# crowsonkb/style_transfer2

Hardware: AMD Instinct MI355X
Metric: style-transfer iters/sec @1024px VGG19 (higher is better)
Workload: dtype f32; 1 GPU; configs[1]: 1024x1024 single image per GPU, VGG19 to conv5_1, content conv4_2 + 5 style layers, adam fp32, 500 iterations per image; jobs=1, parallelism=independent jobs, 1 per GPU, no collective (replicas)

## Files before the change

style_transfer2_amd/csrc/conv3x3_winograd.hip:

```cpp
#include <hip/hip_runtime.h>
#include <stdint.h>
#include <stdlib.h>
#include <string.h>
#include <type_traits>
#include "st2_kernels.h"
#include "env.h"

namespace st2 {

typedef float f32x16 __attribute__((ext_vector_type(16)));
typedef float f32x4 __attribute__((ext_vector_type(4)));


constexpr int WN_CH = 8;
constexpr int WN_IW = 40;
constexpr int WN_V = 4 * 16 * 64;

size_t wino_pack_floats(int K, int M) { return (size_t)((M + 127) / 128 * 4) * (K / 2) * 1024; }

static void wino_pack(const float* w, int Cout, int Cin, bool dgrad, float* dst)
{
    const int K = dgrad ? Cout : Cin, M = dgrad ? Cin : Cout, nkp = K / 2;
    memset(dst, 0, wino_pack_floats(K, M) * sizeof(float));
    static const double G[4][3] = {{1, 0, 0}, {0.5, 0.5, 0.5}, {0.5, -0.5, 0.5}, {0, 0, 1}};
    for (int m = 0; m < M; ++m)
        for (int k = 0; k < K; ++k) {
            double g[3][3], t[4][3], u[4][4];
            for (int tap = 0; tap < 9; ++tap)
                g[tap / 3][tap % 3] = dgrad ? w[((size_t)k * Cin + m) * 9 + (8 - tap)] : w[((size_t)m * Cin + k) * 9 + tap];
            for (int i = 0; i < 4; ++i)
                for (int j = 0; j < 3; ++j) t[i][j] = G[i][0] * g[0][j] + G[i][1] * g[1][j] + G[i][2] * g[2][j];
            for (int i = 0; i < 4; ++i)
                for (int j = 0; j < 4; ++j) u[i][j] = t[i][0] * G[j][0] + t[i][1] * G[j][1] + t[i][2] * G[j][2];
            const size_t base = ((size_t)(m / 32) * nkp + k / 2) * 1024;
            const int lane = (k & 1) * 32 + (m & 31);
            for (int pos = 0; pos < 16; ++pos)
                dst[base + ((size_t)(pos >> 2) * 64 + lane) * 4 + (pos & 3)] = (float)u[pos >> 2][pos & 3];
        }
}
void pack_wino_weights_fwd(const float* w, int Cout, int Cin, float* dst) { wino_pack(w, Cout, Cin, false, dst); }
void pack_wino_weights_dgrad(const float* w, int Cout, int Cin, float* dst) { wino_pack(w, Cout, Cin, true, dst); }

struct WinoKArgs {
    const float* in; const float4* upack; const float* bias; float* out;
    const float* mask_src; const float* inject;
    int K, M, H, W, nch, tiles_x, tiles_y, n_mtiles, relu;
    unsigned in_bytes, u_bytes;
    float* pool_out; int pool_h, pool_w;
    unsigned char* pool_amap;
    const unsigned char* unpool_amap; unsigned amap_bytes; int ph, pw;
    int splits; float* scratch;
    unsigned long long* stamps;
};

typedef __attribute__((address_space(3))) void* lptr_t;
constexpr unsigned kOOB = 0xffffffffu;

__device__ __forceinline__ float f4c(const float4& v, int i) { return i == 0 ? v.x : i == 1 ? v.y : i == 2 ? v.z : v.w; }

template <int EPI, bool RS> struct WinoEpiOps {
    static constexpr bool E_FWD = EPI == 1 || EPI == 2, E_MASK = EPI == 3;
    static constexpr int NEB = RS ? 2 : 4;
    static constexpr int NG = E_MASK ? 2 * NEB : NEB;
    static constexpr int UNDER = NG < 4 ? NG : 4;
    int mw, dm0, odd;
    bool live, has_inj;
    unsigned row0, plane4, out_bytes;
    float mk[E_MASK ? NEB : 1][E_MASK ? 4 : 1][4], ij[E_FWD ? 1 : NEB][E_FWD ? 1 : 4][4], bs[E_FWD ? NEB : 1][E_FWD ? 4 : 1];

    __device__ __forceinline__ void init(const WinoKArgs& a, int lane, int yw, int x0, int m0, int ph, unsigned plane)
    {
        odd = lane & 1;
        const int gy = yw + 2 * ((lane & 31) >> 4) + odd;
        const int gx4 = x0 + 2 * (lane & 14);
        live = gx4 < a.W && gy < a.H;
        mw = m0 + 4 * (lane >> 5);
        dm0 = RS ? 16 * ph : 0;
        has_inj = a.inject != nullptr;
        plane4 = plane * 4u;
        out_bytes = (unsigned)a.M * plane4;
// ... 49 lines not shown
    constexpr int IN_ROWS = PROWS + 2;
    constexpr int IW = QUAD ? WN_IW : 64;
    constexpr int COL0 = QUAD ? 3 : 0;
    constexpr int PLANE = IN_ROWS * IW;
    constexpr int UP_ROWS = PROWS / 2 + 2, UP_COLS = 24;
    constexpr int UP_PLANE = UP_ROWS * UP_COLS;
    constexpr int UP_F = WN_CH * UP_PLANE;
    constexpr int UP_FQ = UP_F / 256, UP_AQ = UP_F / 256;
    static_assert(!UNPOOL || (UP_F % 256 == 0 && NW == 4), "unpool staging is a whole number of wave-DMAs");
    constexpr int N_RAW = UNPOOL ? UP_F + UP_F / 4 : WN_CH * PLANE;
    constexpr int I_PER_WAVE = UNPOOL ? (UP_FQ + UP_AQ + NW - 1) / NW
                             : QUAD ? (N_RAW / 4 + 64 * NW - 1) / (64 * NW) : WN_CH * IN_ROWS / 4;
    constexpr int RAW = UNPOOL ? 1024 : QUAD ? I_PER_WAVE * NW * 256 : N_RAW;
    static_assert(QUAD || (WN_CH * IN_ROWS) % 4 == 0, "rows divide over the four waves");

    __shared__ __attribute__((aligned(16))) float raw_s[2][RAW];
    __shared__ __attribute__((aligned(16))) float v_s[2][TG][WN_V];
    __shared__ __attribute__((aligned(16))) float x8_own[W8 ? 8 * 8 * 64 * 4 : 4];
    static_assert(!H4 || 4 * 8 * 64 * 4 <= 2 * TG * WN_V, "H4: the exchange buffer fits the V images");
    float* const x8_s = H4 ? &v_s[0][0][0] : x8_own;

    const int tid = threadIdx.x;
    const int lane = tid & 63;
    const int wave = __builtin_amdgcn_readfirstlane(tid >> 6);
    const int wave_m = W8 ? (wave & 3) : H4 ? (wave & 1) : wave / TG, wave_g = RS ? 0 : wave % TG;
    const int ph = W8 ? wave >> 2 : H4 ? wave >> 1 : wave_g;

    const int nwg = gridDim.x / a.splits;
    const int split = blockIdx.x / nwg, orig = blockIdx.x - split * nwg;
    const int nch = a.nch / a.splits, c_first = split * nch;
    const int xcd = orig & 7, q = nwg >> 3, r = nwg & 7;
    const int logical = (xcd < r ? xcd * (q + 1) : r * (q + 1) + (xcd - r) * q) + (orig >> 3);
    const int n_pt = a.tiles_x * a.tiles_y;
    const int mt = logical / n_pt;
    const int pt = logical - mt * n_pt;
    const int tx = pt % a.tiles_x;
    const int ty = pt / a.tiles_x;
    const int y0 = ty * PROWS, x0 = tx * 32;
    const unsigned plane = (unsigned)a.H * a.W;
    const int nkp = a.K >> 1;

    const unsigned long long t_begin = DIAG ? __builtin_amdgcn_s_memtime() : 0ull;

    const __amdgpu_buffer_rsrc_t rs_i = __builtin_amdgcn_make_buffer_rsrc((void*)a.in, 0, a.in_bytes, 0x00020000);
    const __amdgpu_buffer_rsrc_t rs_a = __builtin_amdgcn_make_buffer_rsrc((void*)(UNPOOL ? a.unpool_amap : nullptr), 0, UNPOOL ? a.amap_bytes : 0u, 0x00020000);
    const unsigned pplane = UNPOOL ? (unsigned)a.ph * a.pw : 0u;
    unsigned ioff[QUAD ? I_PER_WAVE : 1];
    if (UNPOOL) {
#pragma unroll
        for (int t = 0; t < I_PER_WAVE; ++t) {
            const int piece = wave + NW * t;
            const bool bytes = piece >= UP_FQ;
            const int e = ((bytes ? piece - UP_FQ : piece) * 64 + lane) * 4;
            const int c = e / UP_PLANE;
            const int rem = e - c * UP_PLANE;
            const int rr = rem / UP_COLS;
            const int col = rem - rr * UP_COLS;
            const int gy = (y0 >> 1) - 1 + rr, gx = (x0 >> 1) - 4 + col;
            const bool ok = piece < UP_FQ + UP_AQ && gy >= 0 && gy < a.ph && gx >= 0 && gx + 3 < a.pw;
            ioff[t] = ok ? ((unsigned)((BIG && !bytes ? 0 : c_first * WN_CH) + c) * pplane + (unsigned)gy * a.pw + gx) * (bytes ? 1u : 4u) : kOOB;
        }
    } else if (QUAD) {
#pragma unroll
        for (int t = 0; t < I_PER_WAVE; ++t) {
            const int e = ((wave + NW * t) * 64 + lane) * 4;
            const int c = e / PLANE;
            const int rem = e - c * PLANE;
            const int rr = rem / IW;
            const int col = rem - rr * IW;
            const int gy = y0 - 1 + rr, gx = x0 - 4 + col;
            const bool ok = e < N_RAW && gy >= 0 && gy < a.H && gx >= 0 && gx + 3 < a.W;
            ioff[t] = ok ? ((unsigned)((BIG ? 0 : c_first * WN_CH) + c) * plane + (unsigned)gy * a.W + gx) * 4u : kOOB;
        }
    } else {
        const int gx = x0 - 1 + lane;
        ioff[0] = (lane < 34 && gx >= 0 && gx < a.W) ? (unsigned)gx * 4u : kOOB;
    }
    auto dma_raw = [&](int ch, int buf) {
        const __amdgpu_buffer_rsrc_t rs_c = BIG ? __builtin_amdgcn_make_buffer_rsrc(
            (void*)(a.in + (size_t)(c_first + ch) * WN_CH * (UNPOOL ? pplane : plane)), 0, a.in_bytes, 0x00020000) : rs_i;
        if (UNPOOL) {
#pragma unroll
            for (int t = 0; t < I_PER_WAVE; ++t) {
                const int piece = wave + NW * t;
                if (piece < UP_FQ) {
                    const unsigned vo = (ioff[t] == kOOB || BIG) ? ioff[t] : ioff[t] + (unsigned)ch * WN_CH * pplane * 4u;
                    __builtin_amdgcn_raw_ptr_buffer_load_lds(rs_c, (lptr_t)(raw_s[buf] + piece * 256), 16, vo, 0, 0, 0);
                } else if (piece < UP_FQ + UP_AQ) {
                    const unsigned vo = ioff[t] == kOOB ? kOOB : ioff[t] + (unsigned)ch * WN_CH * pplane;
                    __builtin_amdgcn_raw_ptr_buffer_load_lds(rs_a, (lptr_t)(raw_s[buf] + UP_F + (piece - UP_FQ) * 64), 4, vo, 0, 0, 0);
                }
            }
        } else if (QUAD) {
            const unsigned coff = BIG ? 0u : (unsigned)ch * WN_CH * plane * 4u;
#pragma unroll
            for (int t = 0; t < I_PER_WAVE; ++t) {
                const unsigned vo = ioff[t] == kOOB ? kOOB : ioff[t] + coff;
                __builtin_amdgcn_raw_ptr_buffer_load_lds(rs_c, (lptr_t)(raw_s[buf] + (wave + NW * t) * 256), 16, vo, 0, 0, 0);
            }
        } else {
#pragma unroll
            for (int t = 0; t < I_PER_WAVE; ++t) {
                const int row = wave + 4 * t;
                const int c = row / IN_ROWS, gy = y0 - 1 + (row - c * IN_ROWS);
                const bool row_ok = gy >= 0 && gy < a.H;
                const unsigned base = ((unsigned)((c_first + ch) * WN_CH + c) * plane + (unsigned)(row_ok ? gy : 0) * a.W) * 4u;
                const unsigned vo = (row_ok && ioff[0] != kOOB) ? ioff[0] + base : kOOB;
                __builtin_amdgcn_raw_ptr_buffer_load_lds(rs_i, (lptr_t)(raw_s[buf] + row * 64), 4, vo, 0, 0, 0);
            }
        }
    };

    const int xt = tid & 31, xch = (tid >> 5) & 7;
    const int x_raw = UNPOOL ? xch * UP_PLANE + (xt >> 4) * UP_COLS + (xt & 15) + 3
                             : xch * PLANE + (2 * (xt >> 4)) * IW + 2 * (xt & 15) + COL0;
    const int x_v = (((xch >> 1) * 4) * 64 + (xch & 1) * 32 + xt) * 4;
    float d[TG][16];
    auto pin = [&]() {
#pragma unroll
        for (int g = 0; g < TG; ++g) {
            asm volatile("" : "+v"(d[g][0]), "+v"(d[g][1]), "+v"(d[g][2]), "+v"(d[g][3]), "+v"(d[g][4]), "+v"(d[g][5]), "+v"(d[g][6]), "+v"(d[g][7]));
            asm volatile("" : "+v"(d[g][8]), "+v"(d[g][9]), "+v"(d[g][10]), "+v"(d[g][11]), "+v"(d[g][12]), "+v"(d[g][13]), "+v"(d[g][14]), "+v"(d[g][15]));
        }
    };
    float up_v[UNPOOL ? 9 : 1];
    unsigned up_m[UNPOOL ? 9 : 1];
    auto up_expand = [&]() {
        if constexpr (UNPOOL) {
#pragma unroll
            for (int i = 0; i < 4; ++i)
// ... 47 lines not shown
            for (int i = 0; i < 4; ++i)
                *reinterpret_cast<float4*>(vp + g * WN_V + i * 256) = make_float4(d[g][4 * i], d[g][4 * i + 1], d[g][4 * i + 2], d[g][4 * i + 3]);
    };

    const f32x4* up = reinterpret_cast<const f32x4*>(a.upack) + ((size_t)(mt * WM + wave_m) * nkp + 4 * c_first) * 256 + lane;
    constexpr int UQ = SPLIT ? 2 : 4;
    f32x4 ua[4][UQ];
    auto u_fill = [&](int kp) {
#pragma unroll
        for (int g = 0; g < UQ; ++g) ua[kp & 3][g] = up[((size_t)kp * 4 + (SPLIT ? 2 * ph + g : g)) * 64];
        asm volatile("" ::: "memory");
    };
    auto u_pin = [&](int set) {
        if constexpr (SPLIT) asm volatile("" : "+v"(ua[set][0]), "+v"(ua[set][1]));
        else asm volatile("" : "+v"(ua[set][0]), "+v"(ua[set][1]), "+v"(ua[set][2]), "+v"(ua[set][3]));
    };
    constexpr int NACC = RS ? 8 : 16;
    constexpr int NBQ = NACC / 4;
    f32x4 bq[2][NBQ];
    auto b_fetch = [&](int buf, int kpl, int set) {
#pragma unroll
        for (int pg = 0; pg < NBQ; ++pg) {
            const float* vimg = PS ? v_s[buf][pg >> 1] : v_s[buf][wave_g];
            const int quad = PS ? 2 * ph + (pg & 1) : (RS ? 2 * ph + pg : pg);
            bq[set][pg] = *reinterpret_cast<const f32x4*>(vimg + ((kpl * 4 + quad) * 64 + lane) * 4);
        }
    };
    auto b_pin = [&](int set) {
        if constexpr (RS) asm volatile("" : "+v"(bq[set][1]));
        else asm volatile("" : "+v"(bq[set][1]), "+v"(bq[set][2]), "+v"(bq[set][3]));
    };

    f32x16 acc[NACC];
#pragma unroll
    for (int p = 0; p < NACC; ++p)
#pragma unroll
        for (int e = 0; e < 16; ++e) acc[p][e] = 0.f;

    dma_raw(0, 0);
    if (nch > 1) dma_raw(1, 1);
    u_fill(0); u_fill(1); u_fill(2);
    __syncthreads();
    if (!W8 || ph == 0) {
        xf_read(raw_s[0] + x_raw);
        up_expand();
        xf_math();
        xf_write(&v_s[0][0][0] + x_v);
    }
    __syncthreads();
    b_fetch(0, 0, 0);

    unsigned long long t0 = 0, r0 = 0;
    if (DIAG) { t0 = __builtin_amdgcn_s_memtime(); r0 = __builtin_amdgcn_s_memrealtime(); }

    WinoEpiOps<EPI, RS> eo;
    if constexpr (EPI != 0) eo.init(a, lane, y0 + 4 * wave_g, x0, mt * BM + wave_m * 32, ph, plane);

    auto chunk = [&](const int c, auto more_t, auto more2_t) {
        constexpr bool MORE = decltype(more_t)::value, MORE2 = decltype(more2_t)::value;
        const int cur = c & 1;
        const bool do_xf = !W8 || ph == ((c + 1) & 1);
#pragma unroll
        for (int kpl = 0; kpl < 4; ++kpl) {
            const int kp = 4 * c + kpl;
            const int set = kpl & 1;
#pragma unroll
            for (int p = 0; p < NACC; ++p) {
                acc[p] = __builtin_amdgcn_mfma_f32_32x32x2f32(ua[kpl][SPLIT ? (p >> 2) & 1 : p >> 2][p & 3], bq[set][p >> 2][p & 3], acc[p], 0, 0, 0);
                if (p == 0) {
                    __builtin_amdgcn_sched_barrier(0);
                    b_pin(set);
                    if (kpl < 3) b_fetch(cur, kpl + 1, set ^ 1);
                    else if (MORE) {
                        if constexpr (SPLIT) asm volatile("s_waitcnt vmcnt(4) lgkmcnt(0)\n\ts_barrier" ::: "memory");
                        else asm volatile("s_waitcnt vmcnt(8) lgkmcnt(0)\n\ts_barrier" ::: "memory");
                        b_fetch(cur ^ 1, 0, 0);
                    }
                    if (MORE || kpl == 0) u_fill(kp + 3);
                    if constexpr (EPI != 0) {
                        if constexpr (!MORE) {
                            constexpr int UNDER = WinoEpiOps<EPI, RS>::UNDER;
                            if (kpl >= 4 - UNDER) eo.load(a, kpl - (4 - UNDER));
                        }
                    }
                    if (MORE && do_xf) {
                        if (kpl == 0) xf_read(raw_s[cur ^ 1] + x_raw);
                        if (kpl == 1) { up_expand(); pin(); xf_math(); pin(); }
                        if (kpl == 2) xf_write(&v_s[cur ^ 1][0][0] + x_v);
                    }
// ... 124 lines not shown
            for (int ee = 0; ee < 4; ++ee) { ij[ee][0] = ld2(a.inject, off[ee] + pix0); ij[ee][1] = ld2(a.inject, off[ee] + pix1); }
        }
#pragma unroll
        for (int ee = 0; ee < 4; ++ee) {
            const int e = 4 * eb + ee;
            float o[2][2];
            out_xf(e, o[0][0], o[0][1], o[1][0], o[1][1]);
            if (a.pool_out && live && mb + ee < a.M) {
                float pm = o[0][0];
                if (col1) pm = pm > o[0][1] ? pm : o[0][1];
                if (row1) { pm = pm > o[1][0] ? pm : o[1][0]; if (col1) pm = pm > o[1][1] ? pm : o[1][1]; }
                pm += bs[ee];
                if (relu) pm = pm > 0.f ? pm : 0.f;
                a.pool_out[((size_t)(mb + ee) * a.pool_h + (gy0 >> 1)) * a.pool_w + (gx >> 1)] = pm;
            }
#pragma unroll
            for (int i = 0; i < 2; ++i) {
                float o0 = o[i][0] + bs[ee], o1 = o[i][1] + bs[ee];
                if (relu) { o0 = o0 > 0.f ? o0 : 0.f; o1 = o1 > 0.f ? o1 : 0.f; }
                if (has_mask) { o0 = mk[ee][i].x > 0.f ? o0 : 0.f; o1 = mk[ee][i].y > 0.f ? o1 : 0.f; }
                if (has_inj) { o0 += ij[ee][i].x; o1 += ij[ee][i].y; }
                if (live && mb + ee < a.M && (i == 0 || row1)) {
                    float* dst = outp + off[ee] + (i ? pix1 : pix0);
                    if (wide) *reinterpret_cast<float2*>(dst) = make_float2(o0, o1);
                    else { dst[0] = o0; if (col1) dst[1] = o1; }
                }
            }
        }
    }
  } else if constexpr (EPI != 0) {
    constexpr bool E_FWD = EPI == 1 || EPI == 2, E_POOL = EPI == 2, E_MASK = EPI == 3;
    constexpr int NEB = RS ? 2 : 4;
    typedef unsigned wn_u32x4 __attribute__((ext_vector_type(4)));
    const int t31 = lane & 31;
    const __amdgpu_buffer_rsrc_t rs_o = __builtin_amdgcn_make_buffer_rsrc((void*)a.out, 0, NOOUT ? 0u : eo.out_bytes, 0x00020000);
    const int ty2 = y0 + 4 * wave_g + 2 * (t31 >> 4), tx2 = x0 + 2 * (t31 & 15);
    const bool plive = E_POOL && tx2 < a.W && ty2 < a.H, prow1 = ty2 + 1 < a.H;
    const unsigned pplane = E_POOL ? (unsigned)a.pool_h * a.pool_w : 0u;
    const unsigned ppix = plive ? (unsigned)(ty2 >> 1) * a.pool_w + (tx2 >> 1) : 0u;
    const __amdgpu_buffer_rsrc_t rs_po = __builtin_amdgcn_make_buffer_rsrc((void*)a.pool_out, 0, E_POOL ? (unsigned)a.M * pplane * 4u : 0u, 0x00020000);
    const __amdgpu_buffer_rsrc_t rs_pa = __builtin_amdgcn_make_buffer_rsrc((void*)a.pool_amap, 0, (E_POOL && a.pool_amap) ? (unsigned)a.M * pplane : 0u, 0x00020000);
#pragma unroll
    for (int ebl = 0; ebl < NEB; ++ebl) {
        const int mb = eo.mw + eo.dm0 + 8 * ebl;
        if constexpr (!RS && !E_POOL) {
#pragma unroll
            for (int p = 0; p < NACC; ++p) asm volatile("" : "+a"(acc[p]));
        }
#pragma unroll
        for (int ee = 0; ee < 4; ++ee) {
            const int e = 4 * ebl + ee;
            float y00, y01, y10, y11;
            out_xf(e, y00, y01, y10, y11);
            if constexpr (E_POOL) {
                const float b = eo.bs[E_FWD ? ebl : 0][E_FWD ? ee : 0];
                float pm = y00 > y01 ? y00 : y01;
                const float p1 = y10 > y11 ? y10 : y11, pm2 = pm > p1 ? pm : p1;
                pm = prow1 ? pm2 : pm;
                const float qb = pm + b;
                const unsigned slot = y00 + b == qb ? 0u : (y01 + b == qb ? 1u : (y10 + b == qb ? 2u : 3u));
                const unsigned po = (plive && mb + ee < a.M) ? (unsigned)(mb + ee) * pplane + ppix : kOOB;
                __builtin_amdgcn_raw_buffer_store_b8((unsigned char)(slot | (qb > 0.f ? 4u : 0u)), rs_pa, po, 0, 0);
                pm += b;
                pm = pm > 0.f ? pm : 0.f;
                __builtin_amdgcn_raw_buffer_store_b32(__builtin_bit_cast(unsigned, pm), rs_po, po == kOOB ? kOOB : po * 4u, 0, 0);
            }
            if constexpr (NOOUT) continue;
            const float s0 = eo.odd ? y00 : y10, s1 = eo.odd ? y01 : y11;
            const float r0 = __builtin_bit_cast(float, __builtin_amdgcn_update_dpp(0, __builtin_bit_cast(int, s0), 0xB1, 0xf, 0xf, true));
            const float r1 = __builtin_bit_cast(float, __builtin_amdgcn_update_dpp(0, __builtin_bit_cast(int, s1), 0xB1, 0xf, 0xf, true));
            float o[4];
            o[0] = eo.odd ? r0 : y00; o[1] = eo.odd ? r1 : y01; o[2] = eo.odd ? y10 : r0; o[3] = eo.odd ? y11 : r1;
#pragma unroll
            for (int j = 0; j < 4; ++j) {
                if constexpr (E_FWD) {
                    o[j] += eo.bs[E_FWD ? ebl : 0][E_FWD ? ee : 0];
                    o[j] = o[j] > 0.f ? o[j] : 0.f;
                } else {
                    if constexpr (E_MASK) o[j] = eo.mk[E_MASK ? ebl : 0][E_MASK ? ee : 0][j] > 0.f ? o[j] : 0.f;
                    const float oi = o[j] + eo.ij[E_FWD ? 0 : ebl][E_FWD ? 0 : ee][j];
                    o[j] = eo.has_inj ? oi : o[j];
                }
            }
            wn_u32x4 ov;
#pragma unroll
            for (int j = 0; j < 4; ++j) ov[j] = __builtin_bit_cast(unsigned, o[j]);
            __builtin_amdgcn_raw_buffer_store_b128(ov, rs_o, eo.row_off(a, ebl, ee), 0, 0);
        }
        __builtin_amdgcn_sched_barrier(0);
    }
  } else {
    const int t31 = lane & 31, khalf = lane >> 5;
    const int odd = lane & 1;
    const int gy = y0 + 4 * wave_g + 2 * (t31 >> 4) + odd;
    const int gx4 = x0 + 2 * (t31 & 14);
    const bool part = a.splits > 1;
    const bool has_bias = !part && a.bias != nullptr, has_mask = !part && a.mask_src != nullptr, has_inj = !part && a.inject != nullptr;
    const bool relu = !part && a.relu;
    float* const outp = part ? a.scratch + (size_t)split * a.M * plane : a.out;
    const bool live = gx4 < a.W && gy < a.H;
    const int mw = mt * BM + wave_m * 32 + 4 * khalf;
    const unsigned pix = live ? (unsigned)gy * a.W + gx4 : 0u;
    constexpr int NEB = RS ? 2 : 4;
#pragma unroll
    for (int ebl = 0; ebl < NEB; ++ebl) {
        const int eb = RS ? 2 * ph + ebl : ebl;
        const int mb = mw + 8 * eb;
        unsigned off[4];
        float4 mk[4], ij[4];
        float bs[4];
#pragma unroll
        for (int ee = 0; ee < 4; ++ee) {
            const int m = mb + ee < a.M ? mb + ee : a.M - 1;
            off[ee] = (unsigned)m * plane + pix;
            bs[ee] = has_bias ? a.bias[m] : 0.f;
        }
        if (has_mask) {
#pragma unroll
            for (int ee = 0; ee < 4; ++ee) mk[ee] = *reinterpret_cast<const float4*>(a.mask_src + off[ee]);
        }
        if (has_inj) {
#pragma unroll
            for (int ee = 0; ee < 4; ++ee) ij[ee] = *reinterpret_cast<const float4*>(a.inject + off[ee]);
// ... 17 lines not shown
                        }
                    }
                    pm += bs[ee];
                    if (relu) pm = pm > 0.f ? pm : 0.f;
                    a.pool_out[po] = pm;
                }
            }
            if constexpr (NOOUT) continue;
            const float s0 = odd ? y00 : y10, s1 = odd ? y01 : y11;
            const float r0 = __builtin_bit_cast(float, __builtin_amdgcn_update_dpp(0, __builtin_bit_cast(int, s0), 0xB1, 0xf, 0xf, true));
            const float r1 = __builtin_bit_cast(float, __builtin_amdgcn_update_dpp(0, __builtin_bit_cast(int, s1), 0xB1, 0xf, 0xf, true));
            float o[4];
            o[0] = odd ? r0 : y00; o[1] = odd ? r1 : y01; o[2] = odd ? y10 : r0; o[3] = odd ? y11 : r1;
#pragma unroll
            for (int j = 0; j < 4; ++j) {
                o[j] += bs[ee];
                if (relu) o[j] = o[j] > 0.f ? o[j] : 0.f;
            }
            if (has_mask) {
                o[0] = mk[ee].x > 0.f ? o[0] : 0.f; o[1] = mk[ee].y > 0.f ? o[1] : 0.f;
                o[2] = mk[ee].z > 0.f ? o[2] : 0.f; o[3] = mk[ee].w > 0.f ? o[3] : 0.f;
            }
            if (has_inj) { o[0] += ij[ee].x; o[1] += ij[ee].y; o[2] += ij[ee].z; o[3] += ij[ee].w; }
            if (live && mb + ee < a.M) *reinterpret_cast<float4*>(outp + off[ee]) = make_float4(o[0], o[1], o[2], o[3]);
        }
    }
  }
    if (DIAG) {
        asm volatile("s_waitcnt vmcnt(0)" ::: "memory");
        const unsigned long long t2 = __builtin_amdgcn_s_memtime();
        if (tid == 0 && a.stamps && blockIdx.x == 300)
            printf("[wino stamps] block 300: prologue %llu, loop %llu, epilogue (stores drained) %llu cycles\n", t0 - t_begin, t_loop_end - t0, t2 - t_loop_end);
    }
}


__global__ __launch_bounds__(256, 1) void conv3x3_wino_f32_128x128(const WinoKArgs a) { conv3x3_wino_body<4, 1>(a); }
__global__ __launch_bounds__(256, 1) void conv3x3_wino_f32_64x256(const WinoKArgs a) { conv3x3_wino_body<2, 2>(a); }
__global__ __launch_bounds__(256, 1) void conv3x3_wino_f32_128x128_anyw(const WinoKArgs a) { conv3x3_wino_body<4, 1, 0, false>(a); }
__global__ __launch_bounds__(256, 1) void conv3x3_wino_f32_64x256_anyw(const WinoKArgs a) { conv3x3_wino_body<2, 2, 0, false>(a); }
__global__ __launch_bounds__(256, 1) void conv3x3_wino_f32_ps64x256(const WinoKArgs a) { conv3x3_wino_body<2, 2, 0, true, true>(a); }
__global__ __launch_bounds__(256, 1) void conv3x3_wino_f32_ps64x256_stamped(const WinoKArgs a) { conv3x3_wino_body<2, 2, 1, true, true>(a); }
__global__ __launch_bounds__(512, 2) void conv3x3_wino_f32_w8_128x128(const WinoKArgs a) { conv3x3_wino_body<4, 1, 0, true, false, true>(a); }
__global__ __launch_bounds__(512, 2) void conv3x3_wino_f32_w8_128x128_stamped(const WinoKArgs a) { conv3x3_wino_body<4, 1, 1, true, false, true>(a); }
__global__ __launch_bounds__(256, 2) void conv3x3_wino_f32_h4_64x128(const WinoKArgs a) { conv3x3_wino_body<2, 1, 0, true, false, false, true>(a); }
__global__ __launch_bounds__(256, 2) void conv3x3_wino_f32_h4_64x128_stamped(const WinoKArgs a) { conv3x3_wino_body<2, 1, 1, true, false, false, true>(a); }
__global__ __launch_bounds__(256, 1) void conv3x3_wino_f32_128x128_unpool(const WinoKArgs a) { conv3x3_wino_body<4, 1, 0, true, false, false, false, true>(a); }
__global__ __launch_bounds__(256, 2) void conv3x3_wino_f32_h4_64x128_unpool(const WinoKArgs a) { conv3x3_wino_body<2, 1, 0, true, false, false, true, true>(a); }
__global__ __launch_bounds__(256, 1) void conv3x3_wino_f32_128x128_noout(const WinoKArgs a) { conv3x3_wino_body<4, 1, 0, true, false, false, false, false, false, true>(a); }
__global__ __launch_bounds__(256, 2) void conv3x3_wino_f32_h4_64x128_noout(const WinoKArgs a) { conv3x3_wino_body<2, 1, 0, true, false, false, true, false, false, true>(a); }
#define ST2_WINO_EPI(NAME, BOUNDS, ...) __global__ __launch_bounds__(256, BOUNDS) void NAME(const WinoKArgs a) { conv3x3_wino_body<__VA_ARGS__>(a); }
ST2_WINO_EPI(conv3x3_wino_f32_128x128_fwd, 1, 4, 1, 0, true, false, false, false, false, false, false, 1)
ST2_WINO_EPI(conv3x3_wino_f32_128x128_pool, 1, 4, 1, 0, true, false, false, false, false, false, false, 2)
ST2_WINO_EPI(conv3x3_wino_f32_128x128_poolonly, 1, 4, 1, 0, true, false, false, false, false, false, true, 2)
ST2_WINO_EPI(conv3x3_wino_f32_128x128_dgm, 1, 4, 1, 0, true, false, false, false, false, false, false, 3)
ST2_WINO_EPI(conv3x3_wino_f32_128x128_dg, 1, 4, 1, 0, true, false, false, false, false, false, false, 4)
ST2_WINO_EPI(conv3x3_wino_f32_128x128_unpool_dgm, 1, 4, 1, 0, true, false, false, false, true, false, false, 3)
ST2_WINO_EPI(conv3x3_wino_f32_h4_64x128_fwd, 2, 2, 1, 0, true, false, false, true, false, false, false, 1)
ST2_WINO_EPI(conv3x3_wino_f32_h4_64x128_pool, 2, 2, 1, 0, true, false, false, true, false, false, false, 2)
ST2_WINO_EPI(conv3x3_wino_f32_h4_64x128_poolonly, 2, 2, 1, 0, true, false, false, true, false, false, true, 2)
ST2_WINO_EPI(conv3x3_wino_f32_h4_64x128_dgm, 2, 2, 1, 0, true, false, false, true, false, false, false, 3)
ST2_WINO_EPI(conv3x3_wino_f32_h4_64x128_dg, 2, 2, 1, 0, true, false, false, true, false, false, false, 4)
ST2_WINO_EPI(conv3x3_wino_f32_h4_64x128_unpool_dgm, 2, 2, 1, 0, true, false, false, true, true, false, false, 3)
#undef ST2_WINO_EPI
__global__ __launch_bounds__(256, 1) void conv3x3_wino_f32_128x128_big(const WinoKArgs a) { conv3x3_wino_body<4, 1, 0, true, false, false, false, false, true>(a); }
__global__ __launch_bounds__(256, 2) void conv3x3_wino_f32_h4_64x128_big(const WinoKArgs a) { conv3x3_wino_body<2, 1, 0, true, false, false, true, false, true>(a); }
// ... 27 lines not shown
hipError_t launch_wino_combine(const float* scratch, int splits, const float* bias, int relu, const float* mask_src, const float* inject,
                               float* out, int M, int H, int W, hipStream_t s)
{
    if (((size_t)H * W) % 4 != 0) return hipErrorInvalidValue;
    const size_t n4 = (size_t)M * H * W / 4;
    const unsigned grid = (unsigned)((n4 + 255) / 256 < 2048 ? (n4 + 255) / 256 : 2048);
    wino_combine_k<<<grid, 256, 0, s>>>(scratch, splits, bias, relu, mask_src, inject, out, M, (unsigned)(H * W));
    return hipGetLastError();
}

int wino_splitk(long long nblk, int nch)
{
    int sp = 1;
    while (nblk * sp * 2 <= 256 && nch % (sp * 2) == 0 && nch / (sp * 2) >= 4 && sp < 16) sp *= 2;
    return sp;
}

namespace {
struct WinoTraits { int bm, prows; bool amap, full, stamped; };
WinoTraits wino_traits(int variant)
{
    switch (variant) {
    case WV_128x128: return {128, 4, true, true, false};
    case WV_H4_64x128: return {64, 4, true, true, false};
    case WV_W8_128x128: return {128, 4, true, false, false};
    case WV_64x256: case WV_PS64x256: return {64, 8, false, false, false};
    case WV_64x256_STAMPED: case WV_PS64x256_STAMPED: return {64, 8, false, false, true};
    case WV_H4_64x128_STAMPED: return {64, 4, false, false, true};
    case WV_128x128_STAMPED: case WV_W8_128x128_STAMPED: return {128, 4, false, false, true};
    default: return {128, 4, false, false, false};
    }
}

int wino_default_variant(int M, int W)
{
    const long long forced = env_int("ST2_WINO_CFG", -1);
    if (forced >= 0) return (int)forced;
    const int pad128 = (M + 127) / 128 * 128, pad64 = (M + 63) / 64 * 64;
    if (W % 4 == 0 && env_on("ST2_WINO_PS")) return WV_PS64x256;
    if (W % 4 == 0 && pad128 <= pad64 && env_on("ST2_WINO_W8")) return WV_W8_128x128;
    if (pad128 <= pad64) return WV_128x128;
    return (W % 4 == 0 && !env_off("ST2_WINO_H4")) ? WV_H4_64x128 : WV_64x256;
}
}

WinoLaunch wino_resolve(int K, int M, int H, int W, int forced_variant)
{
    WinoLaunch w{};
    w.quad = W % 4 == 0;
    int v = forced_variant >= 0 ? forced_variant : wino_default_variant(M, W);
    if (!w.quad) {
        if (v == WV_PS64x256 || v == WV_H4_64x128) v = WV_64x256;
        if (v == WV_W8_128x128) v = WV_128x128;
        if (v == WV_H4_64x128_STAMPED) v = WV_64x256;
    }
    w.variant = (WinoVariant)v;
    const WinoTraits t = wino_traits(v);
    w.bm = t.bm; w.prows = t.prows;
    w.nblk = (long long)((W + 31) / 32) * ((H + t.prows - 1) / t.prows) * ((M + t.bm - 1) / t.bm);
    const bool needs_big = 4ull * K * H * W >= 0xfffffff0ull || 4ull * M * H * W >= 0xfffffff0ull;
    auto big_ok = [&] {
        return w.quad && t.full && 32ull * H * W < 0xfffffff0ull && (unsigned long long)M * H * W <= 0x100000000ull && !env_off("ST2_WINO_BIG");
    };
    w.ok = K >= 8 && K % 8 == 0 && W >= 1 && M >= 48 && H >= 1 && (w.quad || !env_off("ST2_WINO_ANYW")) && (!needs_big || big_ok());
    w.big = needs_big || (env_on("ST2_WINO_FORCE_BIG") && big_ok());
    w.splits = 1;
    if (forced_variant < 0 && w.ok && ((size_t)H * W) % 4 == 0 && !env_off("ST2_WINO_SPLITK")) w.splits = wino_splitk(w.nblk, K / WN_CH);
    w.can_pool = w.ok && w.splits == 1 && !env_off("ST2_WINO_POOL");
    w.pool_amap = w.can_pool && w.quad && H % 2 == 0 && t.amap;
    w.can_skip_out = w.pool_amap && !needs_big && t.full;
    w.can_unpool = w.ok && W % 32 == 0 && H % 2 == 0 && t.full && !env_off("ST2_WINO_UNPOOL");
    return w;
}

namespace {
enum WinoEpi { WE_GENERIC, WE_FWD, WE_FWD_POOL, WE_POOLONLY, WE_DGM, WE_DG };
struct WinoBuild { void (*kernel)(const WinoKArgs); unsigned block; int variant; WinoEpi epi; bool quad, big, unpool, noout; };
const WinoBuild kWinoBuilds[] = {
    {conv3x3_wino_f32_128x128_fwd,            256, WV_128x128,               WE_FWD,      true,  false, false, false},
    {conv3x3_wino_f32_128x128_pool,           256, WV_128x128,               WE_FWD_POOL, true,  false, false, false},
    {conv3x3_wino_f32_128x128_poolonly,       256, WV_128x128,               WE_POOLONLY, true,  false, false, true},
    {conv3x3_wino_f32_128x128_dgm,            256, WV_128x128,               WE_DGM,      true,  false, false, false},
    {conv3x3_wino_f32_128x128_dg,             256, WV_128x128,               WE_DG,       true,  false, false, false},
    {conv3x3_wino_f32_128x128_unpool_dgm,     256, WV_128x128,               WE_DGM,      true,  false, true,  false},
    {conv3x3_wino_f32_h4_64x128_fwd,          256, WV_H4_64x128,             WE_FWD,      true,  false, false, false},
    {conv3x3_wino_f32_h4_64x128_pool,         256, WV_H4_64x128,             WE_FWD_POOL, true,  false, false, false},
    {conv3x3_wino_f32_h4_64x128_poolonly,     256, WV_H4_64x128,             WE_POOLONLY, true,  false, false, true},
    {conv3x3_wino_f32_h4_64x128_dgm,          256, WV_H4_64x128,             WE_DGM,      true,  false, false, false},
    {conv3x3_wino_f32_h4_64x128_dg,           256, WV_H4_64x128,             WE_DG,       true,  false, false, false},
    {conv3x3_wino_f32_h4_64x128_unpool_dgm,   256, WV_H4_64x128,             WE_DGM,      true,  false, true,  false},
    {conv3x3_wino_f32_128x128,                256, WV_128x128,               WE_GENERIC,  true,  false, false, false},
    {conv3x3_wino_f32_128x128_anyw,           256, WV_128x128,               WE_GENERIC,  false, false, false, false},
    {conv3x3_wino_f32_128x128_noout,          256, WV_128x128,               WE_GENERIC,  true,  false, false, true},
    {conv3x3_wino_f32_128x128_unpool,         256, WV_128x128,               WE_GENERIC,  true,  false, true,  false},
    {conv3x3_wino_f32_128x128_big,            256, WV_128x128,               WE_GENERIC,  true,  true,  false, false},
    {conv3x3_wino_f32_128x128_unpool_big,     256, WV_128x128,               WE_GENERIC,  true,  true,  true,  false},
    {conv3x3_wino_f32_h4_64x128,              256, WV_H4_64x128,             WE_GENERIC,  true,  false, false, false},
    {conv3x3_wino_f32_h4_64x128_noout,        256, WV_H4_64x128,             WE_GENERIC,  true,  false, false, true},
    {conv3x3_wino_f32_h4_64x128_unpool,       256, WV_H4_64x128,             WE_GENERIC,  true,  false, true,  false},
    {conv3x3_wino_f32_h4_64x128_big,          256, WV_H4_64x128,             WE_GENERIC,  true,  true,  false, false},
    {conv3x3_wino_f32_h4_64x128_unpool_big,   256, WV_H4_64x128,             WE_GENERIC,  true,  true,  true,  false},
    {conv3x3_wino_f32_64x256,                 256, WV_64x256,                WE_GENERIC,  true,  false, false, false},
    {conv3x3_wino_f32_64x256_anyw,            256, WV_64x256,                WE_GENERIC,  false, false, false, false},
    {conv3x3_wino_f32_ps64x256,               256, WV_PS64x256,              WE_GENERIC,  true,  false, false, false},
    {conv3x3_wino_f32_w8_128x128,             512, WV_W8_128x128,            WE_GENERIC,  true,  false, false, false},
    {conv3x3_wino_f32_128x128_stamped,        256, WV_128x128_STAMPED,       WE_GENERIC,  true,  false, false, false},
    {conv3x3_wino_f32_64x256_stamped,         256, WV_64x256_STAMPED,        WE_GENERIC,  true,  false, false, false},
    {conv3x3_wino_f32_ps64x256_stamped,       256, WV_PS64x256_STAMPED,      WE_GENERIC,  true,  false, false, false},
    {conv3x3_wino_f32_w8_128x128_stamped,     512, WV_W8_128x128_STAMPED,    WE_GENERIC,  true,  false, false, false},
    {conv3x3_wino_f32_h4_64x128_stamped,      256, WV_H4_64x128_STAMPED,     WE_GENERIC,  true,  false, false, false},
};
}

hipError_t launch_conv3x3_wino_cfg(const ConvProblem& p, int variant, hipStream_t s)
{
    const WinoLaunch w = wino_resolve(p.K, p.M, p.H, p.W, variant);
    if (!w.ok || (reinterpret_cast<uintptr_t>(p.in) & 15) != 0) return hipErrorInvalidValue;
    const WinoTraits t = wino_traits(w.variant);
    const bool unpool = p.unpool_amap != nullptr, noout = !p.out;
    WinoKArgs k{};
    k.in = p.in; k.upack = reinterpret_cast<const float4*>(p.wpack); k.bias = p.bias; k.out = p.out;
    k.mask_src = p.mask_src; k.inject = p.inject;
    k.K = p.K; k.M = p.M; k.H = p.H; k.W = p.W; k.nch = p.K / WN_CH;
    k.tiles_x = (p.W + 31) / 32; k.tiles_y = (p.H + w.prows - 1) / w.prows; k.n_mtiles = (p.M + w.bm - 1) / w.bm; k.relu = p.relu;
    k.in_bytes = w.big ? (unsigned)(4ull * WN_CH * p.H * p.W) : (unsigned)(4ull * p.K * p.H * p.W);
    if (unpool) {
        if (p.W % 32 != 0 || p.H % 2 != 0 || p.pool_out) return hipErrorInvalidValue;
        k.unpool_amap = p.unpool_amap; k.ph = p.H / 2; k.pw = p.W / 2;
        k.in_bytes = w.big ? (unsigned)(4ull * WN_CH * k.ph * k.pw) : (unsigned)(4ull * p.K * k.ph * k.pw);
        if ((unsigned long long)p.K * k.ph * k.pw >= 0xfffffff0ull) return hipErrorInvalidValue;
        k.amap_bytes = (unsigned)((unsigned long long)p.K * k.ph * k.pw);
    }
    k.u_bytes = (unsigned)(4ull * wino_pack_floats(p.K, p.M));
    k.stamps = p.stamps;
    if (w.nblk <= 0 || w.nblk > 0x7fffffffLL) return hipErrorInvalidValue;
    k.splits = 1; k.scratch = nullptr;
    k.pool_out = p.pool_out; k.pool_h = (p.H + 1) / 2; k.pool_w = (p.W + 1) / 2;
    k.pool_amap = (p.pool_out && w.quad && t.amap) ? p.pool_amap : nullptr;
    if (w.splits > 1 && p.scratch && p.scratch_floats >= (size_t)w.splits * p.M * p.H * p.W) { k.splits = w.splits; k.scratch = p.scratch; }
    if (k.splits > 1 && (p.pool_out || t.stamped)) return hipErrorInvalidValue;
    if (noout && (!k.pool_out || !k.pool_amap || p.mask_src || p.inject)) return hipErrorInvalidValue;
    const bool fwd = p.bias && p.relu && !p.mask_src && !p.inject, dgr = !p.bias && !p.relu && !p.pool_out;
    const WinoEpi epi = (k.splits > 1 || env_off("ST2_WINO_EPI")) ? WE_GENERIC
                        : fwd ? (noout ? WE_POOLONLY : k.pool_out ? WE_FWD_POOL : WE_FWD)
                        : dgr ? (p.mask_src ? WE_DGM : WE_DG) : WE_GENERIC;
    for (const WinoBuild& b : kWinoBuilds) {
        if (b.variant != w.variant || (b.epi != epi && b.epi != WE_GENERIC) || b.quad != w.quad || b.big != w.big || b.unpool != unpool || b.noout != noout) continue;
        b.kernel<<<dim3((unsigned)(w.nblk * k.splits)), dim3(b.block), 0, s>>>(k);
        const hipError_t e = hipGetLastError();
        if (e != hipSuccess || k.splits == 1) return e;
        return launch_wino_combine(k.scratch, k.splits, p.bias, p.relu, p.mask_src, p.inject, p.out, p.M, p.H, p.W, s);
    }
    return hipErrorInvalidValue;
}

hipError_t launch_conv3x3_wino(const ConvProblem& p, hipStream_t s) { return launch_conv3x3_wino_cfg(p, -1, s); }

}
```

style_transfer2_amd/csrc/st2_kernels.h:

```cpp
#pragma once
#include <hip/hip_runtime.h>
#include <stddef.h>
#include <stdint.h>

#include "emit_plan.h"

namespace st2 {

constexpr int kMaxPartials = 1024;
constexpr int kConvCC = 4;
constexpr int kCoutQuantum = 64;

struct ConvProblem {
    const float* in;
    const float* wpack;
    const float* bias;
    float* out;
    const float* mask_src;
    const float* inject;
    int K, M, MPad, H, W;
    int relu;
    unsigned long long* stamps = nullptr;
    unsigned short* out16 = nullptr;
    float* pool_out = nullptr;
    unsigned char* pool_amap = nullptr;
    const unsigned char* unpool_amap = nullptr;
    float* scratch = nullptr;
    size_t scratch_floats = 0;
};
size_t conv_pack_floats(int K, int M);
int conv_mpad(int M);
void pack_conv_weights_fwd(const float* w , int Cout, int Cin, float* dst);
void pack_conv_weights_dgrad(const float* w , int Cout, int Cin, float* dst);
hipError_t launch_conv3x3(const ConvProblem& p, hipStream_t s);
int conv_num_configs();
const char* conv_config_name(int cfg);
int conv_pick_config(const ConvProblem& p);
hipError_t launch_conv3x3_cfg(const ConvProblem& p, int cfg, hipStream_t s);
size_t wino_pack_floats(int K, int M);
void pack_wino_weights_fwd(const float* w, int Cout, int Cin, float* dst);
void pack_wino_weights_dgrad(const float* w, int Cout, int Cin, float* dst);
enum WinoVariant {
    WV_128x128 = 0, WV_64x256 = 1, WV_PS64x256 = 3, WV_W8_128x128 = 6, WV_H4_64x128 = 8,
    WV_128x128_STAMPED = 2, WV_64x256_STAMPED = 5, WV_PS64x256_STAMPED = 4, WV_W8_128x128_STAMPED = 7, WV_H4_64x128_STAMPED = 9,
};
struct WinoLaunch {
    bool ok;
    WinoVariant variant;
    bool quad, big;
    int bm, prows;
    long long nblk;
    int splits;
    bool can_pool;
    bool pool_amap;
    bool can_skip_out;
    bool can_unpool;
};
WinoLaunch wino_resolve(int K, int M, int H, int W, int forced_variant = -1);
int wino_splitk(long long nblk, int nch);
hipError_t launch_maxpool_bwd_amap(const float* dy, const unsigned char* amap, float* dx, int C, int H, int W, hipStream_t s);
hipError_t launch_conv3x3_wino(const ConvProblem& p, hipStream_t s);
hipError_t launch_conv3x3_wino_cfg(const ConvProblem& p, int variant, hipStream_t s);
hipError_t launch_wino_combine(const float* scratch, int splits, const float* bias, int relu, const float* mask_src, const float* inject,
                               float* out, int M, int H, int W, hipStream_t s);
size_t wino_split_pack_elems(int K, int M);
void pack_wino_split_weights_fwd(const float* w, int Cout, int Cin, unsigned short* dst);
void pack_wino_split_weights_dgrad(const float* w, int Cout, int Cin, unsigned short* dst);
WinoLaunch wino_split_resolve(int K, int M, int H, int W);
hipError_t launch_conv3x3_wino_split(const ConvProblem& p, hipStream_t s);
bool conv_dgrad_first_ok(int Cout, int Cin, int H, int W, bool bf16);
hipError_t launch_conv3x3_dgrad_first(const float* dy, const float* w, float* dx, const float* inject, int Cout, int Cin, int H, int W, hipStream_t s);
bool conv_dgrad_first_strip_ok(int Cout, int Cin, int H, int W);
hipError_t launch_conv3x3_dgrad_first_strip(const float* dy, const float* w, float* dx, const float* inject, int Cout, int Cin, int H, int W, hipStream_t s);
bool conv_dgrad_first_quad_ok(int Cout, int Cin, int H, int W, const float* dy);
hipError_t launch_conv3x3_dgrad_first_quad(const float* dy, const float* w, float* dx, const float* inject, int Cout, int Cin, int H, int W, hipStream_t s);
hipError_t launch_conv3x3_dgrad_first16(const unsigned short* dy16, const float* w_rounded, float* dx, const float* inject, int Cout, int Cin,
                                        int H, int W, hipStream_t s);
size_t conv_first_split_pack_elems(int Cout);
void pack_conv_first_split(const float* w , const float* bias , int Cout, int Cin, unsigned short* dst);
bool conv_first_split_ok(int Cin, int Cout, int H, int W);
hipError_t launch_conv3x3_first_split(const float* x, const unsigned short* wpk, float* out, unsigned short* out16,
                                      int Cin, int Cout, int H, int W, int relu, hipStream_t s, unsigned short* bits_out = nullptr);
bool conv_dgrad_smallM_ok(int Cout, int Cin);
hipError_t launch_conv3x3_dgrad_smallM(const float* dy, const float* w, float* dx, const float* inject,
                                       int Cout, int Cin, int H, int W, hipStream_t s);
hipError_t launch_conv3x3_dgrad_smallM16(const unsigned short* dy16, const float* w_rounded, float* dx, const float* inject,
                                         int Cout, int Cin, int H, int W, hipStream_t s);

struct Conv16Problem {
// ... 216 lines not shown
```

Measured before the change: 143.5 it/s.

## Make Winograd conv blocks walk several tiles, prefetching next tile during epilogue

Makes each Winograd conv workgroup handle a run of consecutive spatial tiles (up to 8, chosen so the grid still has enough blocks) instead of one. The input DMA and weight fill for the next tile are issued before the current tile's epilogue stores, so the load for one tile overlaps the writeback of the previous. This is meant to cut per-block prologue cost and launch/occupancy overheads. In exchange the grid gets smaller, which can hurt load balance, and the kernel keeps more live state across iterations.

```diff
diff --git a/style_transfer2_amd/csrc/conv3x3_winograd.hip b/style_transfer2_amd/csrc/conv3x3_winograd.hip
--- a/style_transfer2_amd/csrc/conv3x3_winograd.hip
+++ b/style_transfer2_amd/csrc/conv3x3_winograd.hip
@@ -45,7 +45,8 @@
     const float* in; const float4* upack; const float* bias; float* out;
     const float* mask_src; const float* inject;
     int K, M, H, W, nch, tiles_x, tiles_y, n_mtiles, relu;
-    unsigned in_bytes, u_bytes;
+    unsigned in_bytes;
+    int walk, n_wk;
     float* pool_out; int pool_h, pool_w;
     unsigned char* pool_amap;
     const unsigned char* unpool_amap; unsigned amap_bytes; int ph, pw;
@@ -161,11 +162,14 @@
     const int xcd = orig & 7, q = nwg >> 3, r = nwg & 7;
     const int logical = (xcd < r ? xcd * (q + 1) : r * (q + 1) + (xcd - r) * q) + (orig >> 3);
     const int n_pt = a.tiles_x * a.tiles_y;
-    const int mt = logical / n_pt;
-    const int pt = logical - mt * n_pt;
+    constexpr bool WALK = EPI != 0;
+    const int n_wk = WALK ? a.n_wk : n_pt;
+    const int mt = logical / n_wk;
+    int pt = WALK ? (logical - mt * n_wk) * a.walk : logical - mt * n_pt;
     const int tx = pt % a.tiles_x;
     const int ty = pt / a.tiles_x;
-    const int y0 = ty * PROWS, x0 = tx * 32;
+    [[maybe_unused]] const int pt_end = WALK ? (pt + a.walk < n_pt ? pt + a.walk : n_pt) : pt + 1;
+    int y0 = ty * PROWS, x0 = tx * 32;
     const unsigned plane = (unsigned)a.H * a.W;
     const int nkp = a.K >> 1;
 
@@ -175,10 +179,16 @@
     const __amdgpu_buffer_rsrc_t rs_a = __builtin_amdgcn_make_buffer_rsrc((void*)(UNPOOL ? a.unpool_amap : nullptr), 0, UNPOOL ? a.amap_bytes : 0u, 0x00020000);
     const unsigned pplane = UNPOOL ? (unsigned)a.ph * a.pw : 0u;
     unsigned ioff[QUAD ? I_PER_WAVE : 1];
+    constexpr bool UP_TMAJOR = UNPOOL && EPI != 0;
+    constexpr int UP_TQ = (UP_FQ + NW - 1) / NW;
+    static_assert(!UP_TMAJOR || UP_TQ + (UP_AQ + NW - 1) / NW <= I_PER_WAVE, "unpool: the rounds of both kinds fit");
+    auto up_piece = [](int t, int wave) { return UP_TMAJOR ? (t < UP_TQ ? wave + NW * t : UP_FQ + wave + NW * (t - UP_TQ)) : wave + NW * t; };
+    auto tile_ioff = [](unsigned (&ioff)[QUAD ? I_PER_WAVE : 1], const WinoKArgs& a, const int y0, const int x0, const int lane, const int wave,
+                        const int c_first, const unsigned plane, const unsigned pplane, const bool on, auto up_piece) {
     if (UNPOOL) {
 #pragma unroll
         for (int t = 0; t < I_PER_WAVE; ++t) {
-            const int piece = wave + NW * t;
+            const int piece = up_piece(t, wave);
             const bool bytes = piece >= UP_FQ;
             const int e = ((bytes ? piece - UP_FQ : piece) * 64 + lane) * 4;
             const int c = e / UP_PLANE;
@@ -186,7 +196,7 @@
             const int rr = rem / UP_COLS;
             const int col = rem - rr * UP_COLS;
             const int gy = (y0 >> 1) - 1 + rr, gx = (x0 >> 1) - 4 + col;
-            const bool ok = piece < UP_FQ + UP_AQ && gy >= 0 && gy < a.ph && gx >= 0 && gx + 3 < a.pw;
+            const bool ok = on && piece < (UP_TMAJOR && t < UP_TQ ? UP_FQ : UP_FQ + UP_AQ) && gy >= 0 && gy < a.ph && gx >= 0 && gx + 3 < a.pw;
             ioff[t] = ok ? ((unsigned)((BIG && !bytes ? 0 : c_first * WN_CH) + c) * pplane + (unsigned)gy * a.pw + gx) * (bytes ? 1u : 4u) : kOOB;
         }
     } else if (QUAD) {
@@ -198,25 +208,27 @@
             const int rr = rem / IW;
             const int col = rem - rr * IW;
             const int gy = y0 - 1 + rr, gx = x0 - 4 + col;
-            const bool ok = e < N_RAW && gy >= 0 && gy < a.H && gx >= 0 && gx + 3 < a.W;
+            const bool ok = on && e < N_RAW && gy >= 0 && gy < a.H && gx >= 0 && gx + 3 < a.W;
             ioff[t] = ok ? ((unsigned)((BIG ? 0 : c_first * WN_CH) + c) * plane + (unsigned)gy * a.W + gx) * 4u : kOOB;
         }
     } else {
         const int gx = x0 - 1 + lane;
         ioff[0] = (lane < 34 && gx >= 0 && gx < a.W) ? (unsigned)gx * 4u : kOOB;
     }
-    auto dma_raw = [&](int ch, int buf) {
+    };
+    tile_ioff(ioff, a, y0, x0, lane, wave, c_first, plane, pplane, true, up_piece);
+    auto dma_raw = [&](int ch, int buf, const bool on = true) {
         const __amdgpu_buffer_rsrc_t rs_c = BIG ? __builtin_amdgcn_make_buffer_rsrc(
             (void*)(a.in + (size_t)(c_first + ch) * WN_CH * (UNPOOL ? pplane : plane)), 0, a.in_bytes, 0x00020000) : rs_i;
         if (UNPOOL) {
 #pragma unroll
             for (int t = 0; t < I_PER_WAVE; ++t) {
-                const int piece = wave + NW * t;
-                if (piece < UP_FQ) {
-                    const unsigned vo = (ioff[t] == kOOB || BIG) ? ioff[t] : ioff[t] + (unsigned)ch * WN_CH * pplane * 4u;
+                const int piece = up_piece(t, wave);
+                if (UP_TMAJOR ? t < UP_TQ && piece < UP_FQ : piece < UP_FQ) {
+                    const unsigned vo = !on ? kOOB : (ioff[t] == kOOB || BIG) ? ioff[t] : ioff[t] + (unsigned)ch * WN_CH * pplane * 4u;
                     __builtin_amdgcn_raw_ptr_buffer_load_lds(rs_c, (lptr_t)(raw_s[buf] + piece * 256), 16, vo, 0, 0, 0);
-                } else if (piece < UP_FQ + UP_AQ) {
-                    const unsigned vo = ioff[t] == kOOB ? kOOB : ioff[t] + (unsigned)ch * WN_CH * pplane;
+                } else if ((!UP_TMAJOR || t >= UP_TQ) && piece < UP_FQ + UP_AQ) {
+                    const unsigned vo = (ioff[t] == kOOB || !on) ? kOOB : ioff[t] + (unsigned)ch * WN_CH * pplane;
                     __builtin_amdgcn_raw_ptr_buffer_load_lds(rs_a, (lptr_t)(raw_s[buf] + UP_F + (piece - UP_FQ) * 64), 4, vo, 0, 0, 0);
                 }
             }
@@ -224,7 +236,7 @@
             const unsigned coff = BIG ? 0u : (unsigned)ch * WN_CH * plane * 4u;
 #pragma unroll
             for (int t = 0; t < I_PER_WAVE; ++t) {
-                const unsigned vo = ioff[t] == kOOB ? kOOB : ioff[t] + coff;
+                const unsigned vo = (ioff[t] == kOOB || !on) ? kOOB : ioff[t] + coff;
                 __builtin_amdgcn_raw_ptr_buffer_load_lds(rs_c, (lptr_t)(raw_s[buf] + (wave + NW * t) * 256), 16, vo, 0, 0, 0);
             }
         } else {
@@ -338,14 +350,30 @@
     };
 
     f32x16 acc[NACC];
-#pragma unroll
-    for (int p = 0; p < NACC; ++p)
-#pragma unroll
-        for (int e = 0; e < 16; ++e) acc[p][e] = 0.f;
+    if constexpr (!WALK) {
+#pragma unroll
+        for (int p = 0; p < NACC; ++p)
+#pragma unroll
+            for (int e = 0; e < 16; ++e) acc[p][e] = 0.f;
+    }
 
     dma_raw(0, 0);
     if (nch > 1) dma_raw(1, 1);
-    u_fill(0); u_fill(1); u_fill(2);
+    constexpr bool U_EARLY = WALK && !RS && !UNPOOL && !NOOUT && (EPI == 1 || EPI == 4);
+    if constexpr (U_EARLY) { u_fill(0); u_fill(1); u_fill(2); }
+    WinoEpiOps<EPI, RS> eo;
+  for (;;) {
+    if constexpr (!U_EARLY) { u_fill(0); u_fill(1); u_fill(2); }
+    if constexpr (WALK) {
+#pragma unroll
+        for (int p = 0; p < NACC; ++p)
+#pragma unroll
+            for (int e = 0; e < 16; ++e) acc[p][e] = 0.f;
+        if constexpr (!RS) {
+#pragma unroll
+            for (int p = 0; p < NACC; ++p) asm volatile("" : "+a"(acc[p]));
+        }
+    }
     __syncthreads();
     if (!W8 || ph == 0) {
         xf_read(raw_s[0] + x_raw);
@@ -359,8 +387,9 @@
     unsigned long long t0 = 0, r0 = 0;
     if (DIAG) { t0 = __builtin_amdgcn_s_memtime(); r0 = __builtin_amdgcn_s_memrealtime(); }
 
-    WinoEpiOps<EPI, RS> eo;
-    if constexpr (EPI != 0) eo.init(a, lane, y0 + 4 * wave_g, x0, mt * BM + wave_m * 32, ph, plane);
+    int lane_t = lane;
+    if constexpr (WALK) asm volatile("" : "+v"(lane_t));
+    if constexpr (EPI != 0) eo.init(a, lane_t, y0 + 4 * wave_g, x0, mt * BM + wave_m * 32, ph, plane);
 
     auto chunk = [&](const int c, auto more_t, auto more2_t) {
         constexpr bool MORE = decltype(more_t)::value, MORE2 = decltype(more2_t)::value;
@@ -551,7 +580,16 @@
     constexpr bool E_FWD = EPI == 1 || EPI == 2, E_POOL = EPI == 2, E_MASK = EPI == 3;
     constexpr int NEB = RS ? 2 : 4;
     typedef unsigned wn_u32x4 __attribute__((ext_vector_type(4)));
-    const int t31 = lane & 31;
+    int lane_n = lane;
+    asm volatile("" : "+v"(lane_n));
+    const int t31 = lane_n & 31;
+    const bool has_next = pt + 1 < pt_end;
+    const int ny0 = (pt + 1) / a.tiles_x * PROWS, nx0 = (pt + 1) % a.tiles_x * 32;
+    tile_ioff(ioff, a, ny0, nx0, lane_n, wave, c_first, plane, pplane, has_next, up_piece);
+    dma_raw(0, 0);
+    dma_raw(1, 1, nch > 1);
+    if constexpr (U_EARLY) { u_fill(0); u_fill(1); u_fill(2); }
+    __builtin_amdgcn_sched_barrier(0);
     const __amdgpu_buffer_rsrc_t rs_o = __builtin_amdgcn_make_buffer_rsrc((void*)a.out, 0, NOOUT ? 0u : eo.out_bytes, 0x00020000);
     const int ty2 = y0 + 4 * wave_g + 2 * (t31 >> 4), tx2 = x0 + 2 * (t31 & 15);
     const bool plive = E_POOL && tx2 < a.W && ty2 < a.H, prow1 = ty2 + 1 < a.H;
@@ -608,6 +646,10 @@
         }
         __builtin_amdgcn_sched_barrier(0);
     }
+    if (!has_next) break;
+    asm volatile("s_nop 0");
+    ++pt; y0 = ny0; x0 = nx0;
+    continue;
   } else {
     const int t31 = lane & 31, khalf = lane >> 5;
     const int odd = lane & 1;
@@ -691,6 +733,8 @@
         if (tid == 0 && a.stamps && blockIdx.x == 300)
             printf("[wino stamps] block 300: prologue %llu, loop %llu, epilogue (stores drained) %llu cycles\n", t0 - t_begin, t_loop_end - t0, t2 - t_loop_end);
     }
+    break;
+  }
 }
 
 
@@ -784,6 +828,16 @@
     }
 }
 
+constexpr int kWinoMaxWalk = 8;
+int wino_walk(long long tiles, int n_mtiles, bool half_tile)
+{
+    const long long forced = env_int("ST2_WINO_WALK", 0);
+    if (forced >= 1) return (int)(forced < tiles ? forced : tiles);
+    int walk = 1;
+    while (!half_tile && walk * 2 <= kWinoMaxWalk && walk * 2 <= tiles && (tiles + walk * 2 - 1) / (walk * 2) * n_mtiles >= 256) walk *= 2;
+    return walk;
+}
+
 int wino_default_variant(int M, int W)
 {
     const long long forced = env_int("ST2_WINO_CFG", -1);
@@ -822,6 +876,7 @@
     w.pool_amap = w.can_pool && w.quad && H % 2 == 0 && t.amap;
     w.can_skip_out = w.pool_amap && !needs_big && t.full;
     w.can_unpool = w.ok && W % 32 == 0 && H % 2 == 0 && t.full && !env_off("ST2_WINO_UNPOOL");
+    w.walk = (w.ok && t.full) ? wino_walk(w.nblk / ((M + t.bm - 1) / t.bm), (M + t.bm - 1) / t.bm, v == WV_H4_64x128) : 1;
     return w;
 }
 
@@ -883,7 +938,6 @@
         if ((unsigned long long)p.K * k.ph * k.pw >= 0xfffffff0ull) return hipErrorInvalidValue;
         k.amap_bytes = (unsigned)((unsigned long long)p.K * k.ph * k.pw);
     }
-    k.u_bytes = (unsigned)(4ull * wino_pack_floats(p.K, p.M));
     k.stamps = p.stamps;
     if (w.nblk <= 0 || w.nblk > 0x7fffffffLL) return hipErrorInvalidValue;
     k.splits = 1; k.scratch = nullptr;
@@ -898,7 +952,11 @@
                         : dgr ? (p.mask_src ? WE_DGM : WE_DG) : WE_GENERIC;
     for (const WinoBuild& b : kWinoBuilds) {
         if (b.variant != w.variant || (b.epi != epi && b.epi != WE_GENERIC) || b.quad != w.quad || b.big != w.big || b.unpool != unpool || b.noout != noout) continue;
-        b.kernel<<<dim3((unsigned)(w.nblk * k.splits)), dim3(b.block), 0, s>>>(k);
+        k.walk = b.epi != WE_GENERIC ? w.walk : 1;
+        const long long n_pt = (long long)k.tiles_x * k.tiles_y;
+        k.n_wk = (int)((n_pt + k.walk - 1) / k.walk);
+        const long long grid = b.epi != WE_GENERIC ? (long long)k.n_wk * k.n_mtiles : w.nblk * k.splits;
+        b.kernel<<<dim3((unsigned)grid), dim3(b.block), 0, s>>>(k);
         const hipError_t e = hipGetLastError();
         if (e != hipSuccess || k.splits == 1) return e;
         return launch_wino_combine(k.scratch, k.splits, p.bias, p.relu, p.mask_src, p.inject, p.out, p.M, p.H, p.W, s);
diff --git a/style_transfer2_amd/csrc/st2_kernels.h b/style_transfer2_amd/csrc/st2_kernels.h
--- a/style_transfer2_amd/csrc/st2_kernels.h
+++ b/style_transfer2_amd/csrc/st2_kernels.h
@@ -55,6 +55,7 @@
     bool pool_amap;
     bool can_skip_out;
     bool can_unpool;
+    int walk;
 };
 WinoLaunch wino_resolve(int K, int M, int H, int W, int forced_variant = -1);
 int wino_splitk(long long nblk, int nch);
```

Result: no change. 144.2 it/s, median of 6 (+0.5%).
